# AugmentariumLab/VolumeRenderer

Measured on AMD Instinct MI355X. Metric: Mvoxels/s kd-tree compress+decode, higher is better.
Workload: dtype u8; 1 GPU; 2048x2048x1920 uint8 volume per GPU as 960 bricks of 256x256x128, rm_volume, tolerance 1, maxEpochs 2, VolumeKdtree build + levelCut

## Files before the change

### volumerenderer_amd/csrc/brickset.h

```cpp
#pragma once
#include "kd_common.h"
#include "../../include/vrhip.h"
#include <algorithm>
#include <string>
#include <vector>

namespace vr {

struct Stream2 {
    uint8_t *temp = nullptr;
    uint8_t *codes = nullptr;
    uint8_t *recon[3] = {nullptr, nullptr, nullptr};
    Ctrl *ctrl = nullptr;
    uint8_t *tree = nullptr;
    uint8_t *treeCompact = nullptr;
};

#define EST_R0_BUDGET 8
struct Switches {
    bool decodeWalk = false;
    bool decodeFineV1 = false;
    bool decodeQuad = false;
    bool noSkipBlocks = false;
    bool noUniformBlocks = false;
    bool estExactBounds = false;
    int estBudget = EST_R0_BUDGET;
    bool pyramidBoxes = false;
    bool noUniformDecode = false;
};

#define VR_LOD_SLOTS 4
struct LodSlot {
    int32_t *dev = nullptr;
    int32_t *host = nullptr;
    uint8_t *idxValCut = nullptr;
    uint32_t *decTables = nullptr;
    uint8_t *rankVals = nullptr;
    int64_t *obDev = nullptr;
    int64_t *obHost = nullptr;
    vr_pool_entry *tabHost = nullptr;
    int64_t tabCap = 0;
    hipEvent_t done = nullptr;
    bool pending = false;
};

struct BrickSet {
    int32_t B = 0;
    Switches sw;
    Geom g{};
    TilePlan tile{};
    RegionPlan region{};
    Pyr12Plan pyr12{};
    int32_t D = 0, maxDepth = 0;
    int32_t tolerance = 6, maxEpochs = 5, variant = 0;
    int32_t K = 0;
    int32_t Ds = 0;
    int64_t heapStride = 0;
    int64_t leafStride = 0;
    int64_t codeStride = 0;
    int64_t reconStride = 0;
    bool leafless = false;
    int64_t treeCap = 0;
    int64_t nIdx = 0;

    Stream2 mid, rng;
    uint8_t *mmMin[2] = {nullptr, nullptr}, *mmMax[2] = {nullptr, nullptr};
    unsigned long long *blockErr = nullptr;
    int64_t nErrBlk = 0;
    void *estSumm = nullptr;
    int64_t estSummStride = 0;
    unsigned long long *blockL1 = nullptr;
    uint8_t *blockFlag = nullptr;
    uint8_t *blockFlagR = nullptr;
    uint8_t *blockAlive = nullptr, *blockVal = nullptr;
    unsigned long long *blockSpine = nullptr, *blockSpineR = nullptr;
    uint32_t *chainLut = nullptr;
    uint32_t *blockTot = nullptr, *blockOff = nullptr;
    bool idx64 = false;
    unsigned long long *blockOff64 = nullptr, *idxBase = nullptr;
    int64_t nEmitBlk = 0;
    uint32_t *idxOff = nullptr;
    uint8_t *idxVal = nullptr;
    uint8_t *idxValCut = nullptr;
    uint8_t *fineIdx = nullptr;
    std::vector<uint8_t> fineHas;
    bool fineAll = false;
    uint32_t *decTables = nullptr;
    uint8_t *idxVal3 = nullptr;
    uint32_t *boxUniform = nullptr;
    uint32_t *chainTab = nullptr;
    bool chainTabReady = false;
    std::vector<std::vector<uint8_t>> hostTree;
    uint32_t *lut = nullptr;
    bool foreignRange = false;
    uint32_t *spread = nullptr;
    bool generalGeom = false;
    uint32_t *srcIdx = nullptr;
    uint32_t *ownerRank = nullptr;
    uint8_t *ownerSurv = nullptr;
    uint8_t *rankVals = nullptr;

    std::vector<Ctrl> hostCtrl;
    std::vector<int32_t> hostRevertsR;
    uint32_t lutZeroRun = 0;
    bool encoderReady = false;
    bool built = false, hostCtrlValid = false;
    bool gapped = false;
    bool compactValid = false;
    bool compactOnBuild = true;
    int64_t compactCap = 0;
// ... 50 lines not shown
```

### volumerenderer_amd/csrc/capi.hip

```cpp
#include "../../include/vrhip.h"
#include "brickset.h"
#include "raymarch.h"
#include <math.h>
#include <stdio.h>
#include <stdlib.h>
#include <string.h>
#include <algorithm>
#include <array>
#include <atomic>
#include <map>
#include <mutex>
#include <new>

using namespace vr;

struct vr_brickset { BrickSet s; };

#define HIPCHK(x) do { hipError_t e_ = (x); if (e_ != hipSuccess) return e_ == hipErrorOutOfMemory ? VR_ERR_OOM : VR_ERR_NO_DEVICE; } while (0)

static bool device_ok()
{
    int n = 0;
    hipError_t e = hipGetDeviceCount(&n);
    if ((e != hipSuccess || n <= 0) && getenv("VRHIP_DEBUG"))
// ... 129 lines not shown
        HIPCHK(hipMalloc(&b.mmMax[i], B * (size_t)mm));
    }
    b.nErrBlk = ((int64_t)1 << b.D) / 1024 > 0 ? ((int64_t)1 << b.D) / 1024 : 1;
    HIPCHK(hipMalloc(&b.blockErr, 3 * B * (size_t)b.nErrBlk * sizeof(unsigned long long)));
    b.estSummStride = ((int64_t)1 << b.D) / 1024 > 0 ? ((int64_t)1 << b.D) / 1024 : 1;
    HIPCHK(hipMalloc(&b.estSumm, B * (size_t)b.estSummStride * 128));
    if (b.variant == VR_VARIANT_MIDRANGE) {
        HIPCHK(hipMalloc(&b.blockErrR, 3 * B * (size_t)b.nErrBlk * sizeof(unsigned long long)));
        HIPCHK(hipMalloc(&b.estSummR, B * (size_t)b.estSummStride * 128));
    }
    b.nEmitBlk = (((int64_t)1 << b.D) + 255) / 256;
    HIPCHK(hipMalloc(&b.blockL1, B * (size_t)b.nEmitBlk * sizeof(unsigned long long)));
    if (b.D >= 12) HIPCHK(hipMalloc(&b.blockFlag, B * ((size_t)1 << (b.D - 12))));
    if (b.D >= 12 && b.variant == VR_VARIANT_MIDRANGE) HIPCHK(hipMalloc(&b.blockFlagR, B * ((size_t)1 << (b.D - 12))));
    HIPCHK(hipMalloc(&b.blockAlive, B * (size_t)b.nEmitBlk));
    HIPCHK(hipMalloc(&b.blockVal, B * (size_t)b.nEmitBlk));
    HIPCHK(hipMalloc(&b.blockSpine, B * (size_t)b.nEmitBlk * sizeof(unsigned long long)));
    if (b.variant == VR_VARIANT_MIDRANGE) HIPCHK(hipMalloc(&b.blockSpineR, B * (size_t)b.nEmitBlk * sizeof(unsigned long long)));
    HIPCHK(hipMalloc(&b.chainLut, (260 + 512) * sizeof(uint32_t)));
    HIPCHK(hipMalloc(&b.blockTot, B * (size_t)b.nEmitBlk * sizeof(uint32_t)));
    HIPCHK(hipMalloc(&b.blockOff, B * (size_t)b.nEmitBlk * sizeof(uint32_t)));
    if (b.idx64) {
        HIPCHK(hipMalloc(&b.blockOff64, B * (size_t)b.nEmitBlk * sizeof(unsigned long long)));
        if (!b.idxBase) HIPCHK(hipMalloc(&b.idxBase, B * (size_t)b.nEmitBlk * sizeof(unsigned long long)));
    }
    return VR_OK;
}

static vr_status ensure_encoder_buffers(BrickSet &b)
{
    if (b.encoderReady) return VR_OK;
    const vr_status rc = alloc_encoder_buffers(b);
    if (rc != VR_OK) { (void)hipGetLastError(); free_encoder_buffers(b); return rc; }
    b.encoderReady = true;
    return VR_OK;
}

vr_status vr_brickset_destroy(vr_brickset *h)
{
    if (!h) return VR_OK;
    BrickSet &b = h->s;
    free_lod_slots(&b);
    hipFree(b.errTable);
    free_encoder_buffers(b);
    free_stream2(b.mid);
    free_stream2(b.rng);
    hipFree(b.brickOff); hipFree(b.compactOverflow);
    hipFree(b.idxOff); hipFree(b.idxVal); hipFree(b.idxValCut); hipFree(b.fineIdx); hipFree(b.idxVal3); hipFree(b.boxUniform); hipFree(b.chainTab); hipFree(b.decTables); hipFree(b.lut); hipFree(b.spread); hipFree(b.srcIdx); hipFree(b.ownerRank); hipFree(b.ownerSurv); hipFree(b.rankVals);
    for (int i = 0; i < 8; ++i) if (b.ev[i]) hipEventDestroy(b.ev[i]);
    if (b.evFork) hipEventDestroy(b.evFork);
    for (int i = 0; i < 3; ++i) { if (b.evJoinN[i]) hipEventDestroy(b.evJoinN[i]); if (b.auxN[i]) hipStreamDestroy(b.auxN[i]); }
    delete h;
    return VR_OK;
}

static bool pow2(int64_t v) { return v > 0 && (v & (v - 1)) == 0; }

static bool misaligned16(const void *p) { return ((uintptr_t)p & 15) != 0; }

vr_status vr_brickset_create(vr_brickset **out, int32_t num_bricks, const int64_t dims[3], int32_t tolerance,
                             int32_t max_epochs, int32_t variant)
{
    if (!out || !dims || num_bricks <= 0) return VR_ERR_INVALID;
    if (tolerance < 0 || max_epochs < 0 || variant < 0 || variant > 2) return VR_ERR_INVALID;
    for (int k = 0; k < 3; ++k) if (dims[k] <= 0) return VR_ERR_INVALID;
    if (max_epochs > VR_MAX_EPOCHS) return VR_ERR_UNSUPPORTED;
    bool general = !pow2(dims[0]) || !pow2(dims[1]) || !pow2(dims[2]) || dims[0] > 1024 || dims[1] > 1024 || dims[2] > 1024;
    if (dims[0] > (1ll << 20) || dims[1] > (1ll << 20) || dims[2] > (1ll << 20) || dims[0] * dims[1] * dims[2] >= (1ll << 32))
        return VR_ERR_UNSUPPORTED;
    if (!device_ok()) return VR_ERR_NO_DEVICE;
    vr_brickset *h = new (std::nothrow) vr_brickset();
    if (!h) return VR_ERR_OOM;
    BrickSet &b = h->s;
    b.B = num_bricks;
    {
        Switches &w = b.sw;
        w.decodeWalk = getenv("VRHIP_DECODE_WALK") != nullptr;
        w.decodeFineV1 = getenv("VRHIP_DECODE_FINE_V1") != nullptr;
        w.decodeQuad = getenv("VRHIP_DECODE_QUAD") != nullptr;
        w.noSkipBlocks = getenv("VRHIP_NO_SKIP_BLOCKS") != nullptr;
        w.noUniformBlocks = getenv("VRHIP_NO_UNIFORM_BLOCKS") != nullptr;
        w.noUniformDecode = getenv("VRHIP_NO_UNIFORM_DECODE") != nullptr;
        w.pyramidBoxes = getenv("VRHIP_PYRAMID_BOXES") != nullptr;
        w.estExactBounds = getenv("VRHIP_EST_EXACT_BOUNDS") != nullptr;
        if (const char *eb = getenv("VRHIP_EST_BUDGET")) { const int v = atoi(eb); if (v >= 0) w.estBudget = v; }
    }
    make_geom(b.g, dims);
    b.D = b.g.D;
    if (b.D > 31) { delete h; return VR_ERR_UNSUPPORTED; }
    b.idx64 = b.D > 28 || (getenv("VRHIP_FORCE_IDX64") && b.D >= 12);
    if (b.idx64) general = true;
    if (b.idx64 && num_bricks != 1 && b.D > 28) { delete h; return VR_ERR_UNSUPPORTED; }
    b.generalGeom = general;
    b.maxDepth = b.D + VR_CHAIN_LEVELS;
    b.tolerance = tolerance; b.maxEpochs = max_epochs; b.variant = variant;
    b.K = b.D < 6 ? b.D : 6;
    b.Ds = b.D - b.K;
    b.heapStride = (int64_t)1 << (b.D + 1);
    b.leafStride = (int64_t)1 << b.D;
    b.codeStride = ((b.heapStride + 15) / 16) * 4;
    b.reconStride = b.leafStride;
    const int64_t numMax = b.heapStride - 1 + VR_CHAIN_LEVELS * b.leafStride;
    b.treeCap = ((numMax + 15) / 16 + 2) * 4 + 256;
    if (b.D >= 12) {
        const int64_t gappedBytes = ((int64_t)1 << (b.D - 12)) * 2320 * 4 + 256;
        if (gappedBytes > b.treeCap) b.treeCap = gappedBytes;
    }
    b.nIdx = (int64_t)1 << b.Ds;
    make_plans(b.g, b.K, b.generalGeom, b.idx64, b.treeCap, b.tile, b.region, b.pyr12);
    vr_status rc = alloc_stream2(b, b.mid);
    if (rc == VR_OK) {
        hipError_t e = hipMalloc(&b.idxOff, (size_t)b.B * b.nIdx * sizeof(uint32_t));
        if (e == hipSuccess) e = hipMalloc(&b.idxVal, (size_t)b.B * b.nIdx);
        if (e == hipSuccess) e = hipMalloc(&b.idxValCut, (size_t)b.B * b.nIdx);
        if (e == hipSuccess && general) {
            const int grc = build_general_geometry(&b);
            if (grc != 0) e = grc == -3 ? hipErrorOutOfMemory : hipErrorUnknown;
        }
        const auto upload = [](uint32_t *dst, const std::vector<uint32_t> &v) {
            return hipMemcpy(dst, v.data(), v.size() * sizeof(uint32_t), hipMemcpyHostToDevice);
        };
        if (e == hipSuccess) e = hipMalloc(&b.lut, ((size_t)1 << b.K) * sizeof(uint32_t));
        if (e == hipSuccess && !general) e = upload(b.lut, make_lut(b.g, b.K));
        if (e == hipSuccess && !general) e = hipMalloc(&b.spread, (size_t)(b.g.X + b.g.Y + b.g.Z) * sizeof(uint32_t));
        if (e == hipSuccess && !general) e = upload(b.spread, make_spread(b.g));
        for (int i = 0; i < 8 && e == hipSuccess; ++i) e = hipEventCreate(&b.ev[i]);
        if (e != hipSuccess) rc = e == hipErrorOutOfMemory ? VR_ERR_OOM : VR_ERR_NO_DEVICE;
    }
    if (rc != VR_OK) { vr_brickset_destroy(h); return rc; }
    b.hostCtrl.resize(b.B);
    b.openTreeBytes.assign(b.B, -1);
    *out = h;
    return VR_OK;
}

vr_status vr_brickset_set_switch(vr_brickset *h, const char *name, int32_t value)
{
    if (!h || !name) return VR_ERR_INVALID;
    Switches &w = h->s.sw;
    const bool on = value != 0;
    if (!strcmp(name, "decode_walk")) w.decodeWalk = on;
    else if (!strcmp(name, "decode_fine_v1")) w.decodeFineV1 = on;
    else if (!strcmp(name, "decode_quad")) w.decodeQuad = on;
    else if (!strcmp(name, "no_skip_blocks")) w.noSkipBlocks = on;
    else if (!strcmp(name, "no_uniform_blocks")) w.noUniformBlocks = on;
    else if (!strcmp(name, "no_uniform_decode")) w.noUniformDecode = on;
    else if (!strcmp(name, "pyramid_boxes")) w.pyramidBoxes = on;
    else if (!strcmp(name, "est_exact_bounds")) w.estExactBounds = on;
    else return VR_ERR_INVALID;
    return VR_OK;
}

vr_status vr_brickset_set_compaction(vr_brickset *h, int32_t on_build)
{
    if (!h) return VR_ERR_INVALID;
    h->s.compactOnBuild = on_build != 0;
    return VR_OK;
}

vr_status vr_debug_set(const char *name, int32_t value)
{
    if (!name) return VR_ERR_INVALID;
    if (!strcmp(name, "skip_grid_v1")) { vr::g_skipGridV1.store(value ? 1 : 0); return VR_OK; }
    if (!strcmp(name, "reslice_tile_w")) {
        if (value != 8 && value != 16 && value != 64) return VR_ERR_INVALID;
        vr::g_resliceTileLog2.store(value == 8 ? 3 : (value == 16 ? 4 : 6));
        return VR_OK;
    }
    if (!strcmp(name, "hist_plain")) { vr::g_histPlain.store(value ? 1 : 0); return VR_OK; }
    return VR_ERR_INVALID;
}

vr_status vr_brickset_set_error_tolerance(vr_brickset *h, int32_t tol)
{
    if (!h || tol < 0) return VR_ERR_INVALID;
    h->s.tolerance = tol;
    return VR_OK;
}
vr_status vr_brickset_set_max_epochs(vr_brickset *h, int32_t e)
{
    if (!h || e < 0) return VR_ERR_INVALID;
    if (e > VR_MAX_EPOCHS) return VR_ERR_UNSUPPORTED;
    h->s.maxEpochs = e;
    return VR_OK;
}

vr_status vr_brickset_build(vr_brickset *h, const uint8_t *vox, void *stream)
{
    if (!h || !vox) return VR_ERR_INVALID;
    BrickSet &b = h->s;
    if (build_loads_vectors(&b) && misaligned16(vox)) return VR_ERR_INVALID;
    if (b.encoderReady && b.leafless != leafless_build(b)) {
        HIPCHK(hipDeviceSynchronize());
        free_encoder_buffers(b);
    }
    vr_status rc = ensure_encoder_buffers(b);
    if (rc != VR_OK) return rc;
    b.hostCtrlValid = false;
    b.hostBrickOff.clear();
    b.foreign = false;
    std::fill(b.openTreeBytes.begin(), b.openTreeBytes.end(), -1);
    {
        const int rc = encode_launch(&b, vox, (hipStream_t)stream);
        if (rc != 0) return rc == -3 ? VR_ERR_OOM : VR_ERR_NO_DEVICE;
    }
    b.built = true;
    b.timingsPending = true;
    b.lastStream = stream;
    return VR_OK;
}

static vr_status sync_ctrl(BrickSet &b)
{
    if (!b.built) return VR_ERR_STATE;
    if (b.hostCtrlValid) return VR_OK;
    HIPCHK(hipStreamSynchronize((hipStream_t)b.lastStream));
    HIPCHK(hipMemcpy(b.hostCtrl.data(), b.mid.ctrl, (size_t)b.B * sizeof(Ctrl), hipMemcpyDeviceToHost));
    b.lutZeroRun = 0;
    if (b.chainLut && !b.foreign) HIPCHK(hipMemcpy(&b.lutZeroRun, b.chainLut + 256, sizeof(uint32_t), hipMemcpyDeviceToHost));
    b.hostRevertsR.assign((size_t)b.B, 0);
    if (b.variant == VR_VARIANT_MIDRANGE && !b.foreign && b.rng.ctrl) {
        std::vector<Ctrl> r((size_t)b.B);
        HIPCHK(hipMemcpy(r.data(), b.rng.ctrl, (size_t)b.B * sizeof(Ctrl), hipMemcpyDeviceToHost));
        for (int i = 0; i < b.B; ++i) b.hostRevertsR[(size_t)i] = r[(size_t)i].constBrick ? 0 : r[(size_t)i].numReverts;
    }
    b.hostCtrlValid = true;
    return VR_OK;
}

vr_status vr_brickset_info(vr_brickset *h, int32_t brick, vr_tree_info *info)
// ... 960 lines not shown
```

### volumerenderer_amd/csrc/kd_encode.hip

```cpp
#include "brickset.h"
#include <math.h>
#include <stdio.h>
#include <stdlib.h>
#include <string.h>

namespace vr {

#define FILL_NODES_PER_BLOCK 1024
#define EMIT_RANKS_PER_BLOCK 256

template <bool FROM_VOXELS>
__global__ void __launch_bounds__(256)
k_pyramid(Geom g, int dLeaf, int L, const uint8_t *__restrict__ vox, const uint8_t *__restrict__ inMin,
          const uint8_t *__restrict__ inMax, int64_t inStride, uint8_t *__restrict__ temp, int64_t heapStride,
          uint8_t *__restrict__ tempRange, uint8_t *__restrict__ outMin, uint8_t *__restrict__ outMax,
          int64_t outStride, const uint32_t *__restrict__ srcIdx)
{
    __shared__ uint8_t smn[2][1024], smx[2][1024];
    const int brick = blockIdx.y;
    const uint32_t n = 1u << L;
    const uint32_t base = blockIdx.x << L;
    uint8_t *T = temp + (int64_t)brick * heapStride;
    uint8_t *TR = tempRange ? tempRange + (int64_t)brick * heapStride : nullptr;
    for (uint32_t i = threadIdx.x; i < n; i += blockDim.x) {
// ... 2205 lines not shown
    const uint8_t *dmapR = mr ? a.ctrlsR[brick].distanceMap : nullptr;
    const uint32_t n = 1u << a.D;
    const uint32_t r = blockIdx.x * EMIT_RANKS_PER_BLOCK + threadIdx.x;
    for (int i = threadIdx.x; i < EMIT_LDS_WORDS; i += blockDim.x) { W[i] = 0; WR[i] = 0; }
    Owned o;
    o.nSpine = o.nLeaf = 0; o.finalErr = -1; o.aliveAtDs = 0; o.preDs = 0; o.zeroRun = 0;
    if (r < n) o = owned_tokens(Cb, CbR, Tb, TbR, Rl, RlR, a.D, a.maxDepth, a.tol, c.distanceMap, dmapR, a.Ds, r);
    if (o.zeroRun) atomicAdd(&c.zeroRun, 1);
    uint32_t w = o.nSpine + o.nLeaf, tot;
    uint32_t lo = block_excl_scan_u32(w, shw, tot);
    const uint32_t g0 = a.blockOff[(int64_t)brick * a.nEmitBlk + blockIdx.x];
    const uint32_t phase = g0 & 15u;
    if (w) {
        uint32_t pos = phase + lo;
        lds_put(W, pos, (uint32_t)o.spineBits, o.nSpine < 16 ? o.nSpine : 16);
        if (o.nSpine > 16) lds_put(W, pos + 16, (uint32_t)(o.spineBits >> 32), o.nSpine - 16);
        lds_put(W, pos + o.nSpine, o.leafBits, o.nLeaf);
        if (mr) {
            lds_put(WR, pos, (uint32_t)o.spineBitsR, o.nSpine < 16 ? o.nSpine : 16);
            if (o.nSpine > 16) lds_put(WR, pos + 16, (uint32_t)(o.spineBitsR >> 32), o.nSpine - 16);
            lds_put(WR, pos + o.nSpine, o.leafBitsR, o.nLeaf);
        }
    }
    if (r < n && (r & ((1u << a.K) - 1u)) == 0) {
        const uint32_t s = r >> a.K;
        int val = c.distanceMap[0];
        for (int j = 1; j <= a.Ds; ++j) {
            int code = cget(Cb, ((int64_t)1 << j) + (s >> (a.Ds - j)));
            val = apply_code(val, code, c.distanceMap[j]);
        }
        a.idxOff[(int64_t)brick * a.nIdx + s] = o.aliveAtDs ? g0 + lo + (uint32_t)o.preDs : VR_IDX_DEAD;
        a.idxVal[(int64_t)brick * a.nIdx + s] = (uint8_t)val;
    }
    __syncthreads();
    if (tot == 0) return;
    uint32_t *G = (uint32_t *)(a.tree + (int64_t)brick * a.treeCap) + (g0 >> 4);
    uint32_t *GR = mr ? (uint32_t *)(a.treeR + (int64_t)brick * a.treeCap) + (g0 >> 4) : nullptr;
    const uint32_t nw = ((phase + tot - 1) >> 4) + 1;
    for (uint32_t i = threadIdx.x; i < nw; i += blockDim.x) {
        if (i == 0 || i == nw - 1) { if (W[i]) atomicOr(&G[i], W[i]); if (mr && WR[i]) atomicOr(&GR[i], WR[i]); }
        else { G[i] = W[i]; if (mr) GR[i] = WR[i]; }
    }
}

__global__ void __launch_bounds__(256)
k_block_alive(EmitArgs a, int64_t nblk, int sub)
{
    const int brick = blockIdx.y;
    const int64_t blk = (int64_t)blockIdx.x * 256 + threadIdx.x;
    if (blk >= nblk || a.ctrls[brick].constBrick) return;
    const uint8_t *Cb = a.codes + (int64_t)brick * a.codeStride;
    const uint8_t *dmap = a.ctrls[brick].distanceMap;
    const int dl = a.D - sub;
    bool alive = true;
    int val = dmap[0];
    unsigned long long spine = 0, spineR = 0;
    const uint8_t *CbR = a.codesR ? a.codesR + (int64_t)brick * a.codeStride : nullptr;
    int nsp = 0;
    const uint32_t r0 = (uint32_t)blk << sub;
    const int jmin = r0 ? a.D - (__ffs((int)r0) - 1) : 0;
    bool pathAlive = true;
    for (int j = 0; j < dl; ++j) {
        const int code = cget(Cb, ((int64_t)1 << j) + (blk >> (dl - j)));
        if (j > 0) val = apply_code(val, code, dmap[j]);
        if (pathAlive && j >= jmin) {
            spine |= (unsigned long long)code << (2 * nsp);
            if (CbR) spineR |= (unsigned long long)cget(CbR, ((int64_t)1 << j) + (blk >> (dl - j))) << (2 * nsp);
            ++nsp;
        }
        if (code == 3 && pathAlive) {
            alive = ((blk >> (dl - j)) << (dl - j)) == blk;
            pathAlive = false;
        }
    }
    const int64_t o = (int64_t)brick * a.nEmitBlk + blk;
    a.blockAlive[o] = (uint8_t)((alive ? 1 : 0) | (pathAlive ? 2 : 0));
    a.blockVal[o] = (uint8_t)val;
    a.blockSpine[o] = spine | ((unsigned long long)nsp << 56);
    if (CbR) a.blockSpineR[o] = spineR | ((unsigned long long)nsp << 56);
    a.blockTot[o] = (uint32_t)nsp + (pathAlive ? a.blockOff[o] : 0u);
}

__global__ void __launch_bounds__(256)
k_index12(EmitArgs a, uint32_t nblk)
{
    const int brick = blockIdx.y, t = threadIdx.x & 63, D = a.D;
    Ctrl &c = a.ctrls[brick];
    if (c.constBrick) return;
    const uint32_t blk = blockIdx.x * 4u + (threadIdx.x >> 6);
    if (blk >= nblk) return;
    const int64_t bo = (int64_t)brick * a.nEmitBlk + blk;
    const int bflags = a.blockAlive[bo];
    const int bval = a.blockVal[bo];
    const uint32_t s = (blk << 6) + (uint32_t)t;
    const int64_t io = (int64_t)brick * a.nIdx + s;
    const uint8_t *Cb = a.codes + (int64_t)brick * a.codeStride;
    {
        const int64_t nr = ((int64_t)1 << (D - 12)) + blk;
        const uint32_t rootCode = ((uint32_t)Cb[nr >> 2] >> ((int)(nr & 3) * 2)) & 3u;
        if (rootCode == 3u || !(bflags & 2)) {
            a.idxOff[io] = VR_IDX_DEAD;
            if (a.idxBase && t == 0) a.idxBase[bo] = (unsigned long long)blk * PE_TOKENS;
            a.idxVal[io] = (uint8_t)bval;
            *(uint2 *)(a.idxVal3 + io * 8) = make_uint2((uint32_t)bval * 0x01010101u, (uint32_t)bval * 0x01010101u);
            return;
        }
    }
    const uint32_t local = a.idxOff[io];
    uint32_t cb[7];
    int csh[7], dist[7];
#pragma unroll
    for (int q = 0; q < 7; ++q) {
        const int j = D - 12 + q;
        const int64_t ni = ((int64_t)1 << j) + (s >> (6 - q));
        cb[q] = Cb[ni >> 2];
        csh[q] = (int)(ni & 3) * 2;
        dist[q] = c.distanceMap[j];
    }
    const int64_t n5 = ((int64_t)1 << (D - 5)) + 2 * (int64_t)s, n4 = ((int64_t)1 << (D - 4)) + 4 * (int64_t)s,
                  n3 = ((int64_t)1 << (D - 3)) + 8 * (int64_t)s;
    const uint32_t c5 = (uint32_t)Cb[n5 >> 2] >> ((int)(n5 & 3) * 2), c4 = Cb[n4 >> 2], c3 = *(const uint16_t *)(Cb + (n3 >> 2));
    const int dl5 = c.distanceMap[D - 5], dl4 = c.distanceMap[D - 4], dl3 = c.distanceMap[D - 3];
    int val = bval;
#pragma unroll
    for (int q = 0; q < 7; ++q) {
        const int code = (int)((cb[q] >> csh[q]) & 3u);
        val = (D - 12 + q) == 0 ? val : apply_code(val, code, dist[q]);
    }
    const bool root3 = ((cb[6] >> csh[6]) & 3u) == 3u;
    a.idxOff[io] = ((bflags & 2) && local != VR_IDX_DEAD && !root3) ? (a.idxBase ? 0u : blk * (uint32_t)PE_TOKENS) + local : VR_IDX_DEAD;
    if (a.idxBase && t == 0) a.idxBase[bo] = (unsigned long long)blk * PE_TOKENS;
    a.idxVal[io] = (uint8_t)val;
    uint32_t lo3 = 0, hi3 = 0;
#pragma unroll
    for (int i = 0; i < 8; ++i) {
        int v = apply_code(val, (int)((c5 >> (2 * (i >> 2))) & 3u), dl5);
        v = apply_code(v, (int)((c4 >> (2 * (i >> 1))) & 3u), dl4);
        v = apply_code(v, (int)((c3 >> (2 * i)) & 3u), dl3);
        if (i < 4) lo3 |= (uint32_t)v << (8 * i); else hi3 |= (uint32_t)v << (8 * (i - 4));
    }
    *(uint2 *)(a.idxVal3 + io * 8) = make_uint2(lo3, hi3);
}

#define CC_BLOCKS 16
#define CC_BATCH 4
template <bool RANGE>
__global__ void __launch_bounds__(256)
k_concat12(EmitArgs a, const uint8_t *__restrict__ gap, int64_t nblk)
{
    __shared__ unsigned long long g0S[CC_BLOCKS], spineS[CC_BLOCKS];
    __shared__ uint32_t totS[CC_BLOCKS], cntS[CC_BLOCKS];
    __shared__ unsigned long long bwIdx[2 * CC_BLOCKS];
    __shared__ uint32_t bwVal[2 * CC_BLOCKS];
    __shared__ uint32_t chunkPre[CC_BLOCKS + 1];
    __shared__ uint8_t chunkBlk[CC_BLOCKS * (PE_WORDS / 4 + 4)];
    const int brick = blockIdx.y, t = threadIdx.x;
    Ctrl &c = a.ctrls[brick];
    if (c.constBrick) return;
    if (a.brickOff && a.brickOff[gridDim.y] > (unsigned long long)a.compactCap) return;
    const int64_t blk0 = (int64_t)blockIdx.x * CC_BLOCKS;
    const int64_t base = a.brickOff ? (int64_t)a.brickOff[brick] : (int64_t)brick * a.treeCap;
    uint32_t *G0 = (uint32_t *)((RANGE ? a.treeR : a.tree) + base);
    const uint64_t capTok = a.brickOff ? ~0ull >> 2 : (uint64_t)a.treeCap * 4ull;
    if (t < 2 * CC_BLOCKS) { bwIdx[t] = ~0ull; bwVal[t] = 0u; }
    if (t < CC_BLOCKS) {
        const int64_t blk = blk0 + t;
        unsigned long long g0 = 0, sp = 0;
        uint32_t tot = 0, cnt = 0;
        if (blk < nblk) {
            const int64_t bo = (int64_t)brick * a.nEmitBlk + blk;
            const int bflags = a.blockAlive[bo];
            sp = RANGE ? a.blockSpineR[bo] : a.blockSpine[bo];
            g0 = a.blockOff64 ? a.blockOff64[bo] : (unsigned long long)a.blockOff[bo];
            tot = (bflags & 1) ? a.blockTot[bo] : 0u;
            cnt = (bflags & 2) && tot ? tot - (uint32_t)(sp >> 56) : 0u;
            if (tot && g0 + tot + 32ull > capTok) { atomicMax(&c.emitOverflow, 1); tot = 0; cnt = 0; }
        }
        g0S[t] = g0; spineS[t] = sp; totS[t] = tot; cntS[t] = cnt;
    }
    __syncthreads();
    if (t < CC_BLOCKS && totS[t] != 0u && totS[t] <= 32u) {
        const unsigned long long g0 = g0S[t];
        const uint32_t tot = totS[t], cnt = cntS[t];
        const int nsp = (int)(spineS[t] >> 56);
        unsigned long long v = spineS[t] & 0x00FFFFFFFFFFFFFFull;
        if (cnt) {
            const uint32_t *slot = (const uint32_t *)(gap + (int64_t)brick * a.treeCap) + (size_t)(blk0 + t) * PE_WORDS;
            unsigned long long sv = slot[0];
            if (cnt > 16u) sv |= (unsigned long long)slot[1] << 32;
            if (cnt < 32u) sv &= (1ull << (2 * cnt)) - 1ull;
            v |= sv << (2 * nsp);
        }
        const uint32_t sh = (uint32_t)(g0 & 15ull) * 2u;
        const uint64_t w0 = g0 >> 4, wl = (g0 + tot - 1) >> 4;
        const uint32_t x0 = (uint32_t)(v << sh), x1 = (uint32_t)((v << sh) >> 32), x2 = sh ? (uint32_t)(v >> (64u - sh)) : 0u;
        bwIdx[2 * t] = w0; bwVal[2 * t] = x0;
        if (wl == w0 + 1) { bwIdx[2 * t + 1] = wl; bwVal[2 * t + 1] = x1; }
        else if (wl == w0 + 2) { G0[w0 + 1] = x1; bwIdx[2 * t + 1] = wl; bwVal[2 * t + 1] = x2; }
    }
    if (t == 0) {
        uint32_t run = 0;
        for (int i = 0; i < CC_BLOCKS; ++i) {
            chunkPre[i] = run;
            if (totS[i] > 32u) {
                const uint64_t w0 = g0S[i] >> 4, wl = (g0S[i] + totS[i] - 1) >> 4;
                run += (uint32_t)((wl - (w0 & ~3ull)) / 4 + 1);
            }
        }
        chunkPre[CC_BLOCKS] = run;
    }
    __syncthreads();
    const uint32_t nchunkAll = chunkPre[CC_BLOCKS];
    for (int i = 0; i < CC_BLOCKS; ++i)
        for (uint32_t j = chunkPre[i] + (uint32_t)t; j < chunkPre[i + 1]; j += 256u) chunkBlk[j] = (uint8_t)i;
    __syncthreads();
    const uint32_t *gapW = (const uint32_t *)(gap + (int64_t)brick * a.treeCap) + (size_t)blk0 * PE_WORDS;
    for (uint32_t j0 = (uint32_t)t; j0 < nchunkAll; j0 += 256u * CC_BATCH) {
        uint32_t sv[CC_BATCH][5];
#pragma unroll
        for (int k = 0; k < CC_BATCH; ++k) {
            const uint32_t j = j0 + 256u * (uint32_t)k;
#pragma unroll
            for (int m = 0; m < 5; ++m) sv[k][m] = 0u;
            if (j >= nchunkAll) continue;
// ... 349 lines not shown
        hipEventRecord(bs->evFork, st);
        hipStreamWaitEvent(bs->aux, bs->evFork, 0);
        compress_stream(bs, bs->rng, bs->aux, cMin, cMax, rootStride, skR, bs->blockErrR, bs->estSummR);
        hipEventRecord(bs->evJoin, bs->aux);
    }
    int parts = bs->levelLoopStreams;
    if (parts > 4) parts = 4;
    if (mr || B < 16 * parts || parts < 2) parts = 1;
    if (parts > 1) parts = 1 + ensure_aux(bs, parts - 1);
    if (parts > 1) {
        hipEventRecord(bs->evFork, st);
        for (int p = 1; p < parts; ++p) {
            const int b0 = (int)((int64_t)B * p / parts), b1 = (int)((int64_t)B * (p + 1) / parts);
            hipStreamWaitEvent(bs->auxN[p - 1], bs->evFork, 0);
            compress_stream(bs, bs->mid, bs->auxN[p - 1], cMin, cMax, rootStride, sk, bs->blockErr, bs->estSumm, b0, b1 - b0);
            hipEventRecord(bs->evJoinN[p - 1], bs->auxN[p - 1]);
        }
        compress_stream(bs, bs->mid, st, cMin, cMax, rootStride, sk, bs->blockErr, bs->estSumm, 0, (int)((int64_t)B / parts));
        for (int p = 1; p < parts; ++p) hipStreamWaitEvent(st, bs->evJoinN[p - 1], 0);
    } else
    compress_stream(bs, bs->mid, st, cMin, cMax, rootStride, sk, bs->blockErr, bs->estSumm);
    if (forkR) hipStreamWaitEvent(st, bs->evJoin, 0);
    else if (mr) compress_stream(bs, bs->rng, st, cMin, cMax, rootStride, skR, bs->blockErr, bs->estSumm);
    hipEventRecord(bs->ev[2], st);
    dbg_sync(st, "compress");
    hipLaunchKernelGGL(k_chain_lut, dim3(1), dim3(256), 0, st, kernel_tolerance(*bs), bs->maxDepth - D, bs->chainLut);
    ReconBufs rb{{bs->mid.recon[0], bs->mid.recon[1], bs->mid.recon[2]}};
    ReconBufs rbR{{bs->rng.recon[0], bs->rng.recon[1], bs->rng.recon[2]}};
    int pruneFrom = D - 1;
    bs->fineHas.assign((size_t)B, 0);
    fine_has_changed(*bs);
    if (fused) {
        PruneEmitArgs pa;
        pa.sk = sk; pa.skR = skR;
        pa.D = D; pa.tol = kernel_tolerance(*bs); pa.maxDepth = bs->maxDepth; pa.ctrls = bs->mid.ctrl;
        pa.temp = bs->mid.temp; pa.codes = bs->mid.codes;
        pa.heapStride = bs->heapStride; pa.codeStride = bs->codeStride; pa.leafStride = bs->reconStride;
        pa.rb = rb; pa.subTok = bs->blockOff; pa.nEmitBlk = bs->nEmitBlk; pa.blockL1 = bs->blockL1;
        pa.chainLut = bs->chainLut; pa.idxOff = bs->idxOff; pa.nIdx = bs->nIdx;
        if (!bs->fineIdx && hipMalloc(&bs->fineIdx, (size_t)B * bs->nIdx * 16) != hipSuccess) return -3;
        if (!bs->idxVal3 && hipMalloc(&bs->idxVal3, (size_t)B * bs->nIdx * 8) != hipSuccess) return -3;
        const size_t boxBytes = (size_t)B * ((size_t)1 << (D - 12)) * sizeof(uint32_t);
        if (!bs->boxUniform && hipMalloc(&bs->boxUniform, boxBytes) != hipSuccess) return -3;
        if (hipMemsetAsync(bs->boxUniform, 0, boxBytes, st) != hipSuccess) return -1;
        pa.fineIdx = (uint32_t *)bs->fineIdx; pa.boxUniform = bs->boxUniform;
        pa.ctrlsR = mr ? bs->rng.ctrl : nullptr; pa.tempR = mr ? bs->rng.temp : nullptr; pa.codesR = mr ? bs->rng.codes : nullptr;
        pa.rbR = rbR;
        pa.gap = bs->mid.tree; pa.gapR = mr ? bs->rng.tree : nullptr; pa.treeCap = bs->treeCap;
        const dim3 peGrid((unsigned)((int64_t)1 << (D - 12)), B);
        pa.uniformBlocks = skipOn && bs->leafless && !mr && !bs->sw.noUniformBlocks;
        if (pa.uniformBlocks)
            hipLaunchKernelGGL(k_prune_emit12_const, dim3((unsigned)cdiv((int64_t)1 << (D - 12), PEC_BOXES), B), dim3(256), 0, st, pa);
        if (bs->leafless) {
            hipLaunchKernelGGL((k_prune_emit12<false, true>), peGrid, dim3(256), 0, st, pa);
            if (mr) hipLaunchKernelGGL((k_prune_emit12<true, true>), peGrid, dim3(256), 0, st, pa);
        } else {
            hipLaunchKernelGGL((k_prune_emit12<false, false>), peGrid, dim3(256), 0, st, pa);
            if (mr) hipLaunchKernelGGL((k_prune_emit12<true, false>), peGrid, dim3(256), 0, st, pa);
        }
        pruneFrom = D - 13;
        bs->fineHas.assign((size_t)B, 1);
        fine_has_changed(*bs);
    } else
        hipLaunchKernelGGL(k_prune_leaf, dim3(cdiv((int64_t)1 << D, 256), B), dim3(256), 0, st, D, kernel_tolerance(*bs),
                           bs->mid.ctrl, bs->mid.temp, bs->mid.codes, mr ? bs->rng.codes : nullptr, bs->heapStride,
                           bs->codeStride, rb, bs->reconStride, bs->maxDepth, bs->blockL1, bs->nEmitBlk);
    for (int d = pruneFrom; d >= 0; --d)
        hipLaunchKernelGGL(k_prune_level, dim3(cdiv((int64_t)1 << d, 256), B), dim3(256), 0, st, d, bs->mid.ctrl, bs->mid.codes,
                           mr ? bs->rng.codes : nullptr, bs->codeStride);
    hipLaunchKernelGGL(k_fix_chain_distances, dim3(B), dim3(64), 0, st, D, bs->maxDepth, bs->mid.ctrl,
                       mr ? bs->rng.ctrl : nullptr);
    hipEventRecord(bs->ev[3], st);
    dbg_sync(st, "prune");
    EmitArgs a;
    fill_emit_args(bs, a);
    const int64_t nblk = cdiv((int64_t)1 << D, fused ? 4096 : EMIT_RANKS_PER_BLOCK);
    if (fused) hipLaunchKernelGGL(k_block_alive, dim3(cdiv(nblk, 256), B), dim3(256), 0, st, a, nblk, 12);
    else hipLaunchKernelGGL(k_emit_count, dim3((unsigned)nblk, B), dim3(EMIT_RANKS_PER_BLOCK), 0, st, a);
    dbg_sync(st, "block_alive/count");
    hipLaunchKernelGGL(k_emit_scan, dim3(B), dim3(1024), 0, st, a, nblk);
    dbg_sync(st, "emit_scan");
    bs->gapped = fused;
    bs->compactValid = false;
    if (fused) hipLaunchKernelGGL(k_index12, dim3(cdiv(nblk, 4), B), dim3(256), 0, st, a, (uint32_t)nblk);
    else {
        hipLaunchKernelGGL(k_emit_zero, dim3(cdiv(nblk, 256), B), dim3(256), 0, st, a, nblk);
        hipLaunchKernelGGL(k_emit_write, dim3((unsigned)nblk, B), dim3(EMIT_RANKS_PER_BLOCK), 0, st, a);
    }
    hipLaunchKernelGGL(k_emit_stats, dim3(B), dim3(1024), 0, st, a, (int64_t)(D >= 12 ? cdiv((int64_t)1 << D, 1024) : cdiv((int64_t)1 << D, 256)));
    hipLaunchKernelGGL(k_const_finish, dim3(cdiv(bs->nIdx, 256), B), dim3(256), 0, st, D, bs->mid.ctrl, bs->mid.tree,
                       bs->treeCap, bs->idxOff, bs->idxVal, bs->nIdx);
    if (mr) hipLaunchKernelGGL(k_const_finish_range, dim3(B), dim3(64), 0, st, D, bs->rng.ctrl, bs->rng.tree, bs->treeCap);
    if (fused && bs->compactOnBuild) {
        const int rc = compact_launch(bs, st);
        if (rc != 0) return rc;
    }
    hipEventRecord(bs->ev[4], st);
    dbg_sync(st, "emit_write");
    return launch_status("encode");
}

}
```

Measured before the change: 299,000 Mvoxels/s.

## Batch index emission over 32 blocks per workgroup with live-block compaction

Replaces the per-block index12 kernel with a batched version where each workgroup handles 32 emit blocks. It first classifies live and dead blocks into a shared list, fills dead and constant-brick outputs with vector stores, and gives the live blocks to waves with software-prefetched code loads. Because the new kernel already writes constant bricks, the const_finish pass is cut down to a single small launch per brick. The old kernel stays available behind a switch, at the cost of a more complex kernel and a dependency on const_finish no longer filling indices.

```diff
diff --git a/volumerenderer_amd/csrc/brickset.h b/volumerenderer_amd/csrc/brickset.h
--- a/volumerenderer_amd/csrc/brickset.h
+++ b/volumerenderer_amd/csrc/brickset.h
@@ -26,6 +26,7 @@
     bool estExactBounds = false;
     int estBudget = EST_R0_BUDGET;
     bool pyramidBoxes = false;
+    bool indexPerBlock = false;
     bool noUniformDecode = false;
 };
 
diff --git a/volumerenderer_amd/csrc/capi.hip b/volumerenderer_amd/csrc/capi.hip
--- a/volumerenderer_amd/csrc/capi.hip
+++ b/volumerenderer_amd/csrc/capi.hip
@@ -235,6 +235,7 @@
         w.noUniformBlocks = getenv("VRHIP_NO_UNIFORM_BLOCKS") != nullptr;
         w.noUniformDecode = getenv("VRHIP_NO_UNIFORM_DECODE") != nullptr;
         w.pyramidBoxes = getenv("VRHIP_PYRAMID_BOXES") != nullptr;
+        w.indexPerBlock = getenv("VRHIP_INDEX_PER_BLOCK") != nullptr;
         w.estExactBounds = getenv("VRHIP_EST_EXACT_BOUNDS") != nullptr;
         if (const char *eb = getenv("VRHIP_EST_BUDGET")) { const int v = atoi(eb); if (v >= 0) w.estBudget = v; }
     }
@@ -299,6 +300,7 @@
     else if (!strcmp(name, "no_uniform_blocks")) w.noUniformBlocks = on;
     else if (!strcmp(name, "no_uniform_decode")) w.noUniformDecode = on;
     else if (!strcmp(name, "pyramid_boxes")) w.pyramidBoxes = on;
+    else if (!strcmp(name, "index_per_block")) w.indexPerBlock = on;
     else if (!strcmp(name, "est_exact_bounds")) w.estExactBounds = on;
     else return VR_ERR_INVALID;
     return VR_OK;
diff --git a/volumerenderer_amd/csrc/kd_encode.hip b/volumerenderer_amd/csrc/kd_encode.hip
--- a/volumerenderer_amd/csrc/kd_encode.hip
+++ b/volumerenderer_amd/csrc/kd_encode.hip
@@ -2311,7 +2311,7 @@
 }
 
 __global__ void __launch_bounds__(256)
-k_index12(EmitArgs a, uint32_t nblk)
+k_index12_block(EmitArgs a, uint32_t nblk)
 {
     const int brick = blockIdx.y, t = threadIdx.x & 63, D = a.D;
     Ctrl &c = a.ctrls[brick];
@@ -2369,6 +2369,149 @@
         if (i < 4) lo3 |= (uint32_t)v << (8 * i); else hi3 |= (uint32_t)v << (8 * (i - 4));
     }
     *(uint2 *)(a.idxVal3 + io * 8) = make_uint2(lo3, hi3);
+}
+
+__device__ __forceinline__ int idx_step(int v, uint32_t code, int dist)
+{
+    const int m = (int)(code & 1u) - (int)((code >> 1) & 1u);
+    return min(max(v + __mul24(m, dist), 0), 255);
+}
+
+struct IdxLoads {
+    uint32_t local, cb[7], c5, c4, c3;
+};
+
+__device__ __forceinline__ uint64_t idx_first(int D, uint32_t blk, int q) { return ((uint64_t)1 << (D - 12 + q)) + ((uint64_t)blk << q); }
+__device__ __forceinline__ uint32_t idx_off(uint64_t u, uint32_t lane, int q) { return (uint32_t)(u & 3u) + (lane >> (6 - q)); }
+
+__device__ __forceinline__ IdxLoads idx_loads(const EmitArgs &a, const uint8_t *Cb, int64_t io0, uint32_t blk, uint32_t lane)
+{
+    IdxLoads L;
+    const int D = a.D;
+    L.local = a.idxOff[io0 + ((int64_t)blk << 6) + lane];
+#pragma unroll
+    for (int q = 1; q < 7; ++q) {
+        const uint64_t u = idx_first(D, blk, q);
+        L.cb[q] = (Cb + (u >> 2))[idx_off(u, lane, q) >> 2];
+    }
+    L.c5 = (Cb + (((uint64_t)1 << (D - 7)) + ((uint64_t)blk << 5)))[lane >> 1];
+    L.c4 = (Cb + (((uint64_t)1 << (D - 6)) + ((uint64_t)blk << 6)))[lane];
+    L.c3 = ((const uint16_t *)(Cb + (((uint64_t)1 << (D - 5)) + ((uint64_t)blk << 7))))[lane];
+    return L;
+}
+
+#ifndef IDX_BLOCKS
+#define IDX_BLOCKS 32
+#endif
+static_assert(IDX_BLOCKS == 16 || IDX_BLOCKS == 32 || IDX_BLOCKS == 64, "one lane of the first wave per block; whole pieces per thread");
+__global__ void __launch_bounds__(256)
+k_index12(EmitArgs a, uint32_t nblk)
+{
+    __shared__ uint8_t deadS[IDX_BLOCKS], valS[IDX_BLOCKS], rootS[IDX_BLOCKS], listS[IDX_BLOCKS];
+    __shared__ uint32_t distS[10], nLiveS;
+    const int brick = blockIdx.y, t = threadIdx.x, D = a.D;
+    Ctrl &c = a.ctrls[brick];
+    const uint32_t blk0 = blockIdx.x * (uint32_t)IDX_BLOCKS;
+    const uint32_t nb = nblk - blk0 < (uint32_t)IDX_BLOCKS ? nblk - blk0 : (uint32_t)IDX_BLOCKS;
+    const int64_t io0 = (int64_t)brick * a.nIdx;
+    uint4 *const pOff = (uint4 *)(a.idxOff + io0 + ((int64_t)blk0 << 6));
+    uint4 *const pVal = (uint4 *)(a.idxVal + io0 + ((int64_t)blk0 << 6));
+    uint4 *const pVal3 = (uint4 *)(a.idxVal3 + (io0 + ((int64_t)blk0 << 6)) * 8);
+    const uint4 dead4 = make_uint4(VR_IDX_DEAD, VR_IDX_DEAD, VR_IDX_DEAD, VR_IDX_DEAD);
+    if (c.constBrick) {
+        const uint32_t v4 = (uint32_t)(uint8_t)c.constVal * 0x01010101u;
+#pragma unroll
+        for (int k = 0; k < IDX_BLOCKS / 16; ++k) {
+            const uint32_t p = (uint32_t)t + 256u * k;
+            if ((p >> 4) < nb) pOff[p] = dead4;
+        }
+        if (t < IDX_BLOCKS * 4 && ((uint32_t)t >> 2) < nb) pVal[t] = make_uint4(v4, v4, v4, v4);
+        return;
+    }
+    const uint8_t *Cb = a.codes + (int64_t)brick * a.codeStride;
+    if (t < 64) {
+        bool live = false;
+        if ((uint32_t)t < nb) {
+            const uint32_t blk = blk0 + (uint32_t)t;
+            const int64_t bo = (int64_t)brick * a.nEmitBlk + blk;
+            const int bflags = a.blockAlive[bo];
+            const int bval = a.blockVal[bo];
+            const int64_t nr = ((int64_t)1 << (D - 12)) + blk;
+            const uint32_t rootCode = ((uint32_t)Cb[nr >> 2] >> ((int)(nr & 3) * 2)) & 3u;
+            live = !(rootCode == 3u || !(bflags & 2));
+            deadS[t] = live ? 0 : 1;
+            valS[t] = (uint8_t)bval;
+            rootS[t] = (uint8_t)rootCode;
+            if (a.idxBase) a.idxBase[bo] = (unsigned long long)blk * PE_TOKENS;
+        }
+        const unsigned long long lm = __ballot(live);
+        if (live) listS[__popcll(lm & (((unsigned long long)1 << t) - 1ull))] = (uint8_t)t;
+        if (t == 0) nLiveS = (uint32_t)__popcll(lm);
+    } else if (t < 74)
+        distS[t - 64] = c.distanceMap[D - 12 + (t - 64)];
+    __syncthreads();
+    const uint32_t nLive = nLiveS;
+    const uint32_t w = (uint32_t)__builtin_amdgcn_readfirstlane(t >> 6), lane = (uint32_t)t & 63u;
+    IdxLoads cur = {};
+    if (w < nLive) cur = idx_loads(a, Cb, io0, blk0 + (uint32_t)__builtin_amdgcn_readfirstlane((int)listS[w]), lane);
+    if (nLive < nb) {
+#pragma unroll
+        for (int k = 0; k < IDX_BLOCKS / 16; ++k) {
+            const uint32_t p = (uint32_t)t + 256u * k, b = p >> 4;
+            if (b < nb && deadS[b]) pOff[p] = dead4;
+        }
+        if (t < IDX_BLOCKS * 4) {
+            const uint32_t b = (uint32_t)t >> 2;
+            if (b < nb && deadS[b]) { const uint32_t v4 = (uint32_t)valS[b] * 0x01010101u; pVal[t] = make_uint4(v4, v4, v4, v4); }
+        }
+#pragma unroll
+        for (int k = 0; k < IDX_BLOCKS / 8; ++k) {
+            const uint32_t p = (uint32_t)t + 256u * k, b = p >> 5;
+            if (b < nb && deadS[b]) { const uint32_t v4 = (uint32_t)valS[b] * 0x01010101u; pVal3[p] = make_uint4(v4, v4, v4, v4); }
+        }
+    }
+    if (w >= nLive) return;
+    int dist[10];
+#pragma unroll
+    for (int i = 0; i < 10; ++i) dist[i] = __builtin_amdgcn_readfirstlane((int)distS[i]);
+    if (D == 12) dist[0] = 0;
+    const auto entry = [&](const IdxLoads &L, uint32_t b) {
+        const uint32_t blk = blk0 + b;
+        int val = idx_step(valS[b], rootS[b], dist[0]);
+        uint32_t code6 = 0;
+#pragma unroll
+        for (int q = 1; q < 7; ++q) {
+            code6 = L.cb[q] >> ((idx_off(idx_first(D, blk, q), lane, q) & 3u) * 2u);
+            val = idx_step(val, code6, dist[q]);
+        }
+        const uint32_t c5 = L.c5 >> ((lane & 1u) * 4u);
+        const bool root3 = (code6 & 3u) == 3u;
+        const int64_t io = io0 + ((int64_t)blk << 6) + lane;
+        a.idxOff[io] = (L.local != VR_IDX_DEAD && !root3) ? (a.idxBase ? 0u : blk * (uint32_t)PE_TOKENS) + L.local : VR_IDX_DEAD;
+        a.idxVal[io] = (uint8_t)val;
+        int v5[2], v4[4];
+        uint32_t lo3 = 0, hi3 = 0;
+#pragma unroll
+        for (int i = 0; i < 2; ++i) v5[i] = idx_step(val, c5 >> (2 * i), dist[7]);
+#pragma unroll
+        for (int i = 0; i < 4; ++i) v4[i] = idx_step(v5[i >> 1], L.c4 >> (2 * i), dist[8]);
+#pragma unroll
+        for (int i = 0; i < 8; ++i) {
+            const uint32_t v = (uint32_t)idx_step(v4[i >> 1], L.c3 >> (2 * i), dist[9]);
+            if (i < 4) lo3 |= v << (8 * i); else hi3 |= v << (8 * (i - 4));
+        }
+        *(uint2 *)(a.idxVal3 + io * 8) = make_uint2(lo3, hi3);
+    };
+    const auto block_of = [&](uint32_t e) { return (uint32_t)__builtin_amdgcn_readfirstlane((int)listS[e]); };
+    for (uint32_t e = w; e < nLive; e += 8u) {
+        const uint32_t e1 = e + 4u < nLive ? e + 4u : e;
+        const IdxLoads oth = idx_loads(a, Cb, io0, blk0 + block_of(e1), lane);
+        entry(cur, block_of(e));
+        if (e1 == e) break;
+        const uint32_t e2 = e + 8u < nLive ? e + 8u : e1;
+        cur = idx_loads(a, Cb, io0, blk0 + block_of(e2), lane);
+        entry(oth, block_of(e1));
+    }
 }
 
 #define CC_BLOCKS 16
@@ -2884,14 +3027,20 @@
     dbg_sync(st, "emit_scan");
     bs->gapped = fused;
     bs->compactValid = false;
-    if (fused) hipLaunchKernelGGL(k_index12, dim3(cdiv(nblk, 4), B), dim3(256), 0, st, a, (uint32_t)nblk);
+    const bool idxBatched = fused && !bs->sw.indexPerBlock;
+    if (idxBatched) hipLaunchKernelGGL(k_index12, dim3(cdiv(nblk, IDX_BLOCKS), B), dim3(256), 0, st, a, (uint32_t)nblk);
+    else if (fused) hipLaunchKernelGGL(k_index12_block, dim3(cdiv(nblk, 4), B), dim3(256), 0, st, a, (uint32_t)nblk);
     else {
         hipLaunchKernelGGL(k_emit_zero, dim3(cdiv(nblk, 256), B), dim3(256), 0, st, a, nblk);
         hipLaunchKernelGGL(k_emit_write, dim3((unsigned)nblk, B), dim3(EMIT_RANKS_PER_BLOCK), 0, st, a);
     }
     hipLaunchKernelGGL(k_emit_stats, dim3(B), dim3(1024), 0, st, a, (int64_t)(D >= 12 ? cdiv((int64_t)1 << D, 1024) : cdiv((int64_t)1 << D, 256)));
-    hipLaunchKernelGGL(k_const_finish, dim3(cdiv(bs->nIdx, 256), B), dim3(256), 0, st, D, bs->mid.ctrl, bs->mid.tree,
-                       bs->treeCap, bs->idxOff, bs->idxVal, bs->nIdx);
+    if (idxBatched)
+        hipLaunchKernelGGL(k_const_finish, dim3(1, B), dim3(64), 0, st, D, bs->mid.ctrl, bs->mid.tree,
+                           bs->treeCap, bs->idxOff, bs->idxVal, (int64_t)0);
+    else
+        hipLaunchKernelGGL(k_const_finish, dim3(cdiv(bs->nIdx, 256), B), dim3(256), 0, st, D, bs->mid.ctrl, bs->mid.tree,
+                           bs->treeCap, bs->idxOff, bs->idxVal, bs->nIdx);
     if (mr) hipLaunchKernelGGL(k_const_finish_range, dim3(B), dim3(64), 0, st, D, bs->rng.ctrl, bs->rng.tree, bs->treeCap);
     if (fused && bs->compactOnBuild) {
         const int rc = compact_launch(bs, st);
```

Result: faster. 302,700 Mvoxels/s (median of 6 runs) (+1.2%).
